# markokr/libacm

Hardware: AMD Instinct MI355X
Metric: decoded PCM Msamples/sec over a batch of ACM streams (hot path on HBM-resident staged input) (higher is better)
Workload: dtype int32

## Files before the change

libacm_amd/_build.py:

```python
import os
import shutil
import subprocess

ROOT = os.path.dirname(os.path.dirname(os.path.abspath(__file__)))
PKG = os.path.join(ROOT, "libacm_amd")
CSRC = os.path.join(PKG, "csrc")
LIB = os.path.join(PKG, "lib")
BIN = os.path.join(PKG, "bin")
INC = os.path.join(ROOT, "include")

HIPCC = os.environ.get("HIPCC") or shutil.which("hipcc") or "/opt/rocm/bin/hipcc"
GFX = "gfx950"


def _stale(target, sources):
    if not os.path.exists(target):
        return True
    t = os.path.getmtime(target)
    return any(os.path.getmtime(s) > t for s in sources if os.path.exists(s))


def _run(cmd):
    r = subprocess.run(cmd, stdout=subprocess.PIPE, stderr=subprocess.STDOUT, text=True)
    if r.returncode != 0:
        raise RuntimeError("build step failed: %s\n%s" % (" ".join(cmd), r.stdout))
    return r.stdout


def _headers():
    return [os.path.join(INC, f) for f in os.listdir(INC)] + \
           [os.path.join(CSRC, f) for f in os.listdir(CSRC) if f.endswith((".h", ".hpp", ".inc"))]


def build_synth(force=False):
    os.makedirs(LIB, exist_ok=True)
    out = os.path.join(LIB, "libacmsynth.so")
    src = [os.path.join(CSRC, "acm_synth.c")]
    if force or _stale(out, src + _headers()):
        _run(["gcc", "-O2", "-g", "-Wall", "-Wextra", "-fPIC", "-shared", "-I", INC, "-o", out] + src)
    return out


HIP_SOURCES = ["acm_kernels.hip", "acm_kernels_f32.hip", "acm_parse.hip", "acm_hip_api.cpp", "acm_fill.cpp", "acm_pack.cpp", "acm_stream.cpp", "acm_batch.cpp",
               "acm_host_synth.cpp", "acm_plan_cut.cpp", "acm_index.cpp", "acm_batch_windows.cpp", "acm_batch_layout.cpp"]
HOST_ONLY = {"acm_host_synth.cpp", "acm_plan_cut.cpp", "acm_index.cpp", "acm_batch_layout.cpp"}
INCLUDES = {"acm_kernels_f32.hip": ["acm_kernels.hip"]}


def build_hip(force=False):
    os.makedirs(LIB, exist_ok=True)
    out = os.path.join(LIB, "libacm_hip.so")
    src = [os.path.join(CSRC, f) for f in HIP_SOURCES if os.path.exists(os.path.join(CSRC, f))]
    if force or _stale(out, src + _headers()):
        objs = []
        for s in src:
            o = os.path.join(LIB, os.path.basename(s) + ".o")
            deps = [os.path.join(CSRC, f) for f in INCLUDES.get(os.path.basename(s), [])]
            if force or _stale(o, [s] + deps + _headers()):
                cmd = [HIPCC, "-O3", "-g1", "-std=c++17", "-fPIC", "-Wall", "-Wextra",
                       "--offload-arch=" + GFX, "-I", INC, "-I", CSRC, "-c", s, "-o", o]
                if os.environ.get("ACM_ABLATION"):
                    cmd.insert(1, "-DACM_ABLATION=1")
                if os.environ.get("ACM_TUNING"):
                    cmd.insert(1, "-DACM_TUNING=1")
                extra = os.environ.get("ACM_HIPCC_EXTRA", "").split()
                cmd[1:1] = extra
                if os.path.basename(s) in HOST_ONLY:
                    cmd = [c for c in cmd if not c.startswith("--offload-arch")]
                elif s.endswith(".cpp"):
                    cmd.insert(1, "-x")
                    cmd.insert(2, "hip")
                _run(cmd)
            objs.append(o)
        _run([HIPCC, "-shared", "-fPIC", "--offload-arch=" + GFX, "-o", out] + objs + ["-lpthread"])
    return out


def build_tuning(force=False):
# ... 55 lines not shown
```

libacm_amd/csrc/acm_device.h:

```cpp
#ifndef ACM_DEVICE_H
#define ACM_DEVICE_H

#include <stdint.h>

#include "acm_hip.h"

struct AcmDevStream {
	uint64_t idx_off;
	uint64_t hdr_off;
	uint64_t pcm_off;
	uint64_t n_emit;
	uint64_t scratch_off;
	uint32_t level;
	uint32_t rows;
	uint32_t nrows;
	uint32_t row_begin;
	uint32_t halo_row;
	uint32_t pad;
};

struct AcmTile {
	uint32_t stream;
	int32_t row0;
	uint32_t flags;
// ... 85 lines not shown
int acmhip_aux_stream(acmhip_device *dev, int k, void **out);
int acmhip_report_hip(int hip_error, const char *what);
void acmhip_set_error_text(const char *text);

#define ACMK_FMT_F32 0x100u
int acmk_tuning_build(void);
int acmk_warmup(void *stream);
int acmk_fused_variants(void);
int acmk_fused_tile_rows(uint32_t level, int variant);
int acmk_fused_has_carry(uint32_t level, int variant);
int acmk_fused_grid(uint32_t level, int variant, int cus);
int acmk_launch_fused(uint32_t level, int variant, int cus, int carry, const AcmDevStream *d_streams, const AcmTile *d_tiles,
		      uint32_t ntiles, const int16_t *d_idx, const acmhip_blkhdr *d_hdr, int16_t *d_pcm, unsigned fmt, void *stream);
int acmk_tile2_rows(uint32_t level);
int acmk_tile2_grid(uint32_t level, int cus);
#define ACM_K2_SINK_BYTES 65536
#define ACM_K2_SINK_F32_BYTES (2 * ACM_K2_SINK_BYTES)
int acmk_launch_tile2(uint32_t level, int cus, const AcmTile2 *d_tiles, uint32_t ntiles, const int16_t *d_idx, const acmhip_blkhdr *d_hdr, int16_t *d_pcm,
		      int16_t *d_sink, unsigned fmt, void *stream);
int acmk_tile2p_rows(uint32_t level);
int acmk_tile2p_group_rows(uint32_t level);
int acmk_tile2p_slots(uint32_t level);
int acmk_tile2p_waves(uint32_t level);
int acmk_tile2p_pad_shift(uint32_t level);
int acmk_launch_tile2p(uint32_t level, int cus, const AcmTile2 *d_tiles, uint32_t ntiles, const acmhip_packed_chunk *d_chunks, const uint8_t *d_blob,
		       const acmhip_blkhdr *d_hdr, int16_t *d_pcm, int16_t *d_sink, unsigned fmt, void *stream);
int acmk_tile2m_rows(uint32_t level);
int acmk_tile2m_lead_in(uint32_t level);
int acmk_tile2m_run_waves(uint32_t level, int cus);
int acmk_tile2m_grid(uint32_t level, int cus);
int acmk_tile2m_stages(uint32_t level);
int acmk_launch_tile2m(uint32_t level, int cus, const AcmTile2 *d_tiles, uint32_t ntiles, const uint8_t *d_mform, const acmhip_mform_pair *d_pairs,
		       const acmhip_blkhdr *d_hdr, int16_t *d_pcm, int16_t *d_sink, unsigned fmt, void *stream);
int acmk_launch_unpack(const AcmDevStream *d_streams, const uint32_t *d_list, uint32_t nlist, uint64_t max_elems,
		       const int16_t *d_idx, const acmhip_blkhdr *d_hdr, int32_t *d_x, uint32_t shift, void *stream);
int acmk_launch_prefix(const AcmDevStream *d_streams, const uint32_t *d_list, uint32_t nlist, uint64_t max_elems,
		       uint32_t level, const int16_t *d_idx, const acmhip_blkhdr *d_hdr, int32_t *d_y, void *stream);
int acmk_plane_tile_rows(void);
int acmk_plane_grid(int cus);
int acmk_launch_fused_plane(int cus, int carry, const AcmDevStream *d_streams, const AcmTile *d_tiles, uint32_t ntiles,
			    const int32_t *d_plane, int16_t *d_pcm, unsigned fmt, void *stream);
int acmk_launch_patch(const AcmDevPatch *d_patches, uint64_t n, int32_t *d_x, void *stream);
int acmk_launch_stage(const AcmDevStream *d_streams, const uint32_t *d_list, uint32_t nlist, uint64_t max_elems,
		      uint32_t level, uint32_t k, const int32_t *d_in, int32_t *d_out, uint32_t shift, void *stream);
int acmk_parse_supported(uint32_t level, uint32_t rows, uint64_t file_len, uint64_t blocks);
int acmk_launch_parse(const AcmParseJob *d_jobs, uint32_t njobs, const uint8_t *d_files, uint32_t *d_colpos, int16_t *d_idx,
		      acmhip_blkhdr *d_hdr, AcmParseResult *d_res, uint32_t *d_flags, uint64_t max_columns, void *stream);
#define ACM_PARSE_RANGE_MAX_STREAMS 32768
int acmk_launch_parse_range(const AcmParseJob *d_jobs, uint32_t njobs, const uint8_t *d_files, uint32_t *d_colpos, int16_t *d_idx,
			    acmhip_blkhdr *d_hdr, AcmParseResult *d_res, uint32_t *d_flags, uint64_t max_columns, uint32_t r, uint32_t R,
			    uint32_t stripes_up, void *stream);
int acmk_launch_parse_range_mf(const AcmParseJob *d_jobs, uint32_t njobs, const uint8_t *d_files, uint32_t *d_colpos, int16_t *d_idx,
			       acmhip_blkhdr *d_hdr, AcmParseResult *d_res, uint32_t *d_flags, uint64_t max_columns, uint32_t r, uint32_t R,
			       uint32_t stripes_up, uint8_t *d_mf, uint32_t *d_pairs, uint32_t *d_blkoff, void *stream);
int acmk_launch_parse_blocks(const AcmParseJob *d_jobs, uint32_t njobs, const AcmBlockJob *d_bjobs, uint32_t nblock, const uint8_t *d_files,
			     uint32_t *d_colpos, int16_t *d_idx, acmhip_blkhdr *d_hdr, AcmParseResult *d_res, uint32_t *d_flags,
			     uint64_t max_columns, void *stream);
uint32_t acmk_stripe_bound(uint32_t file_len, uint32_t s, uint32_t S);
uint32_t acmk_range_bound(uint32_t blocks, uint32_t r, uint32_t R, uint32_t unit);
int acmk_launch_scatter_stripe(const AcmParseJob *d_jobs, uint32_t njobs, const uint64_t *d_stripe_at, const uint8_t *d_stage,
			       uint8_t *d_files, uint32_t s, uint32_t S, void *stream);
int acmk_launch_small(uint32_t level, const AcmDevStream *d_streams, const uint32_t *d_list, uint32_t nlist, uint64_t max_emit,
		      const int16_t *d_idx, const acmhip_blkhdr *d_hdr, int16_t *d_pcm, unsigned fmt, void *stream);
int acmk_launch_emit(const AcmDevStream *d_streams, const uint32_t *d_list, uint32_t nlist, uint64_t max_emit,
		     const int32_t *d_x, int16_t *d_pcm, unsigned fmt, void *stream);
int acmk_launch_fused_f32(uint32_t level, int variant, int cus, int carry, const AcmDevStream *d_streams, const AcmTile *d_tiles,
// ... 17 lines not shown
```

libacm_amd/csrc/acm_kernels.hip:

```cpp
#include <hip/hip_runtime.h>

#include <utility>

#include "acm_device.h"

#ifndef ACM_L14_GROUPS
#define ACM_L14_GROUPS 3, 3, 3, 3, 2
#endif
#ifndef ACM_L13_GROUPS
#define ACM_L13_GROUPS 2, 3, 3, 3, 2
#endif

#ifndef ACM_OUT_F32
#define ACM_OUT_F32 0
#endif
#if ACM_OUT_F32
#define ACM_K_EMIT acm_sw_emit_f32
#define ACM_K_SMALL acm_small_level_f32
#define ACM_K_FUSED acm_fused_tile_f32
#define ACM_K_TILE2 acm_f32_tile2
#define ACM_K_CHUNK acm_f32_chunk
#define ACMK_OUT(name) name##_f32
#else
#define ACM_K_EMIT acm_sw_emit
#define ACM_K_SMALL acm_small_level
#define ACM_K_FUSED acm_fused_tile
#define ACM_K_TILE2 acm_tile2
#define ACM_K_CHUNK acm_chunk
#define ACMK_OUT(name) name
#endif

namespace {

__device__ __forceinline__ uint32_t pcm16(int32_t v, int level, unsigned fmt)
{
	uint32_t w = (uint32_t)(v >> level);
	if (fmt & 2u)
// ... 1978 lines not shown
#ifndef ACM_K3_DPP_HISTORY
#define ACM_K3_DPP_HISTORY 1
#endif
	static constexpr bool HISTORY_BY_DPP = ACM_K3_DPP_HISTORY && RR >= 2 && NSW == 2 && RR * SIGMA == 16 && SIGMA >= 4;
	static constexpr bool KEEPS_ROWS = HISTORY_IN_REGISTERS || HISTORY_BY_DPP;
	template <int CTRL, int BANKS>
	static __device__ __forceinline__ v4u_t dpp4(const v4u_t old, const v4u_t src)
	{
		v4u_t r;
#pragma unroll
		for (int v = 0; v < 4; v++)
			r[v] = (uint32_t)__builtin_amdgcn_update_dpp((int)old[v], (int)src[v], CTRL, 0xF, BANKS, false);
		return r;
	}
	static constexpr int DPP_W0_BANKS = (1 << (SIGMA / 4)) - 1;
	static __device__ __forceinline__ void hand_history_on(Raw &raw)
	{
#pragma unroll
		for (int k = 0; k < 2; k++) {
			raw.lo[0][k] = dpp4<0x100 + (16 - SIGMA), DPP_W0_BANKS>(raw.lo[0][k], raw.lo[0][k + NSW]);
			raw.hi[0][k] = dpp4<0x100 + (16 - SIGMA), DPP_W0_BANKS>(raw.hi[0][k], raw.hi[0][k + NSW]);
		}
	}
	static __device__ __forceinline__ void take_history_from_partner(Raw &raw)
	{
#pragma unroll
		for (int k = 0; k < 2; k++) {
			raw.lo[0][k] = dpp4<0x110 + SIGMA, 0xF & ~DPP_W0_BANKS>(raw.lo[0][k], raw.lo[0][k + NSW]);
			raw.hi[0][k] = dpp4<0x110 + SIGMA, 0xF & ~DPP_W0_BANKS>(raw.hi[0][k], raw.hi[0][k + NSW]);
		}
	}
	static constexpr int JM = (TR & 1) ? 1 : TR / 2;
	static_assert(JM + 1 <= NE, "entries in reach are entries fetched");
	static __device__ __forceinline__ uint32_t half_bytes(const uint32_t cls) { return (0x4234u >> (4u * cls)) & 15u; }
	template <int J0>
	static __device__ __forceinline__ uint32_t mode_of(const uint32_t flags, const Desc &d, const uint32_t sval)
	{
		const uint32_t cls = d.e[0] & 3u;
		const uint32_t pair_units = (uint32_t)(COLS / 64) * half_bytes(cls);
		bool ok = (flags & ACM_TILE_ONEBLOCK) != 0 && cls != 0u;
		if constexpr (OutScale<L>::SHIFT != 0)
			ok = ok && sval < 65536u;
#pragma unroll
		for (int j = 1; j <= JM; j++)
			ok = ok && (d.e[j] & 3u) == cls;
#pragma unroll
		for (int j = J0; j < JM; j++)
			ok = ok && (d.e[j + 1] >> 2) - (d.e[j] >> 2) == pair_units;
		return ok ? (cls == ACMHIP_BP_NIB12 ? 3u : cls - (ACMHIP_BP_BYTE - 1u)) : 0u;
	}

#ifndef ACM_K3_LD_MOD
#define ACM_K3_LD_MOD " nt"
#endif
	template <bool KEEP>
	static __device__ __forceinline__ void issue(Raw &raw, const uint8_t *arena, const Desc &d, const int lane, const uint32_t odd, const uint32_t mode)
	{
		static_assert(!KEEP || KEEPS_ROWS, "the rows in front belong to another lane");
		constexpr int K0 = KEEP ? 2 : 0, J0 = KEEP ? 1 : 0;
		const uint32_t i = (uint32_t)lane & 15u, ks = (uint32_t)lane >> 4;
		const uint32_t c = class_of(i), rr = RR == 1 ? 0u : i / SIGMA;
		const uint32_t smode = __builtin_amdgcn_readfirstlane(mode);
		uint32_t va[NX][NG], vh[NX][NG];
		const uint8_t *sb[NX][NG];
		if (mode) {
			const uint32_t hb = smode == 1u ? 2u : smode == 2u ? 4u : 3u;
			const uint64_t base = reinterpret_cast<uint64_t>(arena) + ((uint64_t)(d.e[J0] >> 2) << 6);
			const uint32_t vl = (rr * (uint32_t)(NSW * COLS / 2) + c * (uint32_t)(QN / 2)) * hb + 16u * ks;
			const uint32_t vlh = vl - (smode == 3u ? 8u * ks : 0u);
#pragma unroll
			for (int k = K0; k < NX; k++)
#pragma unroll
				for (int g = 0; g < NG; g++) {
					va[k][g] = vl;
					vh[k][g] = vlh;
					sb[k][g] = sgpr_u64(base + (uint64_t)((((TR & 1 ? odd : 0u) + (uint32_t)(k - K0)) * (uint32_t)(COLS / 2) + group_at(g) * (uint32_t)(QN / 2)) * hb));
				}
		} else {
			const uint32_t e0 = d.e[0];
			const uint8_t *base = sgpr_u64(reinterpret_cast<uint64_t>(arena) + ((uint64_t)(e0 >> 2) << 6));
#pragma unroll
			for (int k = K0; k < NX; k++) {
				const uint32_t u = (TR & 1 ? odd : 0u) + rr * NSW + k;
				const uint32_t e = entry_of(d, u);
				const uint32_t hb = half_bytes(e & 3u);
				const uint32_t row_at = (((e >> 2) - (e0 >> 2)) << 6) + ((u & 1u) ? (uint32_t)(COLS / 2) * hb : 0u) + 16u * ks;
#pragma unroll
				for (int g = 0; g < NG; g++) {
					va[k][g] = row_at + (group_at(g) + c) * (uint32_t)(QN / 2) * hb;
					vh[k][g] = va[k][g] - ((e & 3u) == ACMHIP_BP_NIB12 ? 8u * ks : 0u);
					sb[k][g] = base;
				}
			}
		}
#pragma unroll
// ... 40 lines not shown
		for (int g = 0; g < NG; g++)
#pragma unroll
			for (int k = 0; k < 2; k++) {
				raw.lo[g][k] = raw.lo[g][k + NSW];
				raw.hi[g][k] = raw.hi[g][k + NSW];
			}
	}
	static __device__ __forceinline__ void zero_history(Raw &raw)
	{
		const v4u_t z = { 0, 0, 0, 0 };
#pragma unroll
		for (int g = 0; g < NG; g++)
#pragma unroll
			for (int k = 0; k < 2; k++)
				raw.lo[g][k] = raw.hi[g][k] = z;
	}

	static __device__ __forceinline__ v4i_t mfma(const v4u_t data, const v4i_t coef, const v4i_t acc)
	{
		return __builtin_amdgcn_mfma_i32_16x16x64_i8((v4i_t)data, coef, acc, 0, 0, 0);
	}

	static __device__ __forceinline__ int32_t opaque_s(int32_t v)
	{
		asm("" : "+s"(v));
		return v;
	}
	static __device__ __forceinline__ int32_t opaque_v(int32_t v)
	{
		asm("" : "+v"(v));
		return v;
	}

	template <bool WORDS, bool FAST, bool NIB = false>
	static __device__ __forceinline__ void run_t(const Raw &raw, uint32_t *const tile, const Tables &t, const int lane, const uint32_t hvs,
						     const uint32_t in_front, const uint32_t sval, const bool wordu = false, const Desc *dd = nullptr,
						     const uint32_t odd = 0u, const bool nform = false)
	{
		static_assert(!NIB || (WORDS && FAST), "rows in N form are a fast-path matter; the general path takes them to bytes first");
		const v4i_t zero = { 0, 0, 0, 0 };
		const uint32_t h = (uint32_t)lane >> 4, qd = (uint32_t)lane & 15u;
		uint32_t c0[NH], rrd[NH];
		uint32_t o_lane[NH];
#pragma unroll
		for (int hf = 0; hf < NH; hf++) {
			const uint32_t i = 4u * h + (uint32_t)(hf * NVH);
			c0[hf] = RR == 1 ? class_of(i) : i % SIGMA;
			rrd[hf] = RR == 1 ? 0u : i / SIGMA;
			const uint32_t m_lane = rrd[hf] * (uint32_t)(NSW * COLS) + c0[hf] + (uint32_t)SIGMA * qd;
			o_lane[hf] = m_lane + (m_lane >> PS);
		}
		uint32_t bias_at[NSW][NH];
		int32_t val[NSW][NH], dv2[NSW][NH], dv1[NSW][NH];
		bool step2[NSW], step1[NSW];
		bool small[NSW];
#pragma unroll
		for (int s = 0; s < NSW; s++)
			small[s] = OutScale<L>::SHIFT == 0;
		if constexpr (FAST) {
#pragma unroll
			for (int s = 0; s < NSW; s++) {
				step2[s] = step1[s] = false;
				small[s] = true;
#pragma unroll
				for (int hf = 0; hf < NH; hf++)
					val[s][hf] = dv2[s][hf] = dv1[s][hf] = 0;
			}
		} else if constexpr (RR <= 2) {
			int32_t rowval[TR + 2];
#pragma unroll
			for (int k = 0; k < TR + 2; k++)
				rowval[k] = (int32_t)__builtin_amdgcn_readlane(hvs, k);
// ... 18 lines not shown
				}
			}
		} else {
			const uint32_t first = (uint32_t)__builtin_amdgcn_readfirstlane(hvs);
			const bool one_val = __builtin_amdgcn_ballot_w64(lane < TR + 2 && hvs != first) == 0;
#pragma unroll
			for (int s = 0; s < NSW; s++)
				step2[s] = step1[s] = false;
#pragma unroll
			for (int hf = 0; hf < NH; hf++) {
				int32_t g[NSW + 2];
#pragma unroll
				for (int k = 0; k < NSW + 2; k++)
					g[k] = one_val ? (int32_t)first : __builtin_amdgcn_ds_bpermute((int)(4u * (rrd[hf] * NSW + (uint32_t)k)), (int32_t)hvs);
#pragma unroll
				for (int s = 0; s < NSW; s++) {
					val[s][hf] = g[s + 2];
					dv2[s][hf] = g[s + 1] - g[s + 2];
					dv1[s][hf] = g[s] - g[s + 1];
					if (!one_val) {
						step2[s] = step2[s] || __builtin_amdgcn_ballot_w64(dv2[s][hf] != 0) != 0;
						step1[s] = step1[s] || __builtin_amdgcn_ballot_w64(dv1[s][hf] != 0) != 0;
					}
				}
			}
		}
#pragma unroll
		for (int s = 0; s < NSW; s++)
#pragma unroll
			for (int hf = 0; hf < NH; hf++) {
				const uint32_t row = in_front + rrd[hf] * NSW + s;
				bias_at[s][hf] = ((row < 2 ? row : 2u) * 2u + (c0[hf] == 0 ? 0u : 1u)) * (uint32_t)QN + qd;
			}
		const v4i_t *cf = &t.coef[0][0][lane];
		const auto &hi = raw.hi;
#ifndef ACM_K3_MT_UNROLL
#define ACM_K3_MT_UNROLL 1
#endif
#define ACM_PRAGMA_(x) _Pragma(#x)
#define ACM_UNROLL(n) ACM_PRAGMA_(unroll n)
		ACM_UNROLL(ACM_K3_MT_UNROLL)
		for (int mt = 0; mt < NM; mt++) {
			const v4i_t cf0 = cf[0], cf1 = cf[NM * 64], cf2 = cf[2 * NM * 64];
#pragma unroll
			for (int e = 0; e < NSET; e++) {
				const int g = e / NSW, s = e % NSW;
				int32_t b[NH];
#pragma unroll
				for (int hf = 0; hf < NH; hf++)
					b[hf] = g == 0 ? (&t.bias[0][0][0])[bias_at[s][hf] + 16u * (uint32_t)mt] : 0;
				const v4i_t l1 = mfma(raw.lo[g][s], cf2, zero);
				const v4i_t l2 = mfma(raw.lo[g][s + 1], cf1, l1);
				const v4i_t la = mfma(raw.lo[g][s + 2], cf0, l2);
				v4i_t y;
				if constexpr (FAST) {
					const int32_t sv = opaque_s((int32_t)__builtin_amdgcn_readfirstlane(sval));
#pragma unroll
					for (int v = 0; v < 4; v++)
						y[v] = __mul24(la[v], sv) + (v % NVH == 0 ? b[v / NVH] : 0);
					if constexpr (WORDS) {
						const v4i_t h1 = mfma(hi[g][s], cf2, zero);
						const v4i_t h2 = mfma(hi[g][s + 1], cf1, h1);
						const v4i_t ha = mfma(hi[g][s + 2], cf0, h2);
						if constexpr (NIB) {
							const int32_t sv4 = opaque_s((int32_t)__builtin_amdgcn_readfirstlane(sval << 4));
#pragma unroll
							for (int v = 0; v < 4; v++)
								y[v] = __mul24(ha[v], sv4) + y[v];
						} else {
							const uint32_t sv8 = (uint32_t)opaque_s((int32_t)__builtin_amdgcn_readfirstlane(sval << 8));
#pragma unroll
							for (int v = 0; v < 4; v++)
								y[v] = (int32_t)(__umul24((uint32_t)ha[v], sv8) + (uint32_t)y[v]);
						}
					}
				} else {
#pragma unroll
				for (int v = 0; v < 4; v++)
					y[v] = __mul24(la[v], val[s][v / NVH]) + (v % NVH == 0 ? b[v / NVH] : 0);
				if (step2[s]) {
#pragma unroll
					for (int v = 0; v < 4; v++)
						y[v] += __mul24(l2[v], dv2[s][v / NVH]);
				}
				if (step1[s]) {
#pragma unroll
					for (int v = 0; v < 4; v++)
						y[v] += __mul24(l1[v], dv1[s][v / NVH]);
				}
				if constexpr (WORDS && NH == 1) {
					if (wordu) {
						const int32_t *rs = &t.rsum[0][0] + 16 * mt + (int)qd;
						bool urow[3];
#pragma unroll
						for (int j = 0; j < 3; j++)
							urow[j] = (entry_of(*dd, (TR & 1 ? odd : 0u) + rrd[0] * NSW + (uint32_t)(s + j)) & 3u) == ACMHIP_BP_WORDU;
						const int32_t v0 = val[s][0], v1 = v0 + dv2[s][0], v2 = v1 + dv1[s][0];
// ... 38 lines not shown
					}
					if (step1[s]) {
#pragma unroll
						for (int v = 0; v < 4; v++)
							yh[v] += __mul24(h1[v], w1[v / NVH]);
					}
					const uint32_t hs = nform ? 4u : 8u;
#pragma unroll
					for (int v = 0; v < 4; v++)
						y[v] = (int32_t)(((uint32_t)opaque_v(yh[v]) << hs) + (uint32_t)y[v]);
					}
				joined:;
				}
				}
				static_assert(COLS % (1 << PS) == 0 && (SIGMA * 16) % (1 << PS) == 0 &&
					      (NG == 1 || (group_at(NG - 1) % (1 << PS) + CB + 7 < (1 << PS) && SIGMA % (1 << PS) == 0)), "address split");
#pragma unroll
				for (int hf = 0; hf < NH; hf++) {
					uint32_t *const o = tile + (o_lane[hf] + (uint32_t)((s * COLS + ((s * COLS) >> PS)) + (group_at(g) + (group_at(g) >> PS))));
#pragma unroll
					for (int v = 0; v < NVH; v++)
						o[v] = (uint32_t)y[hf * NVH + v];
				}
			}
			cf += 64;
#pragma unroll
			for (int hf = 0; hf < NH; hf++)
				o_lane[hf] += SIGMA * 16 + ((SIGMA * 16) >> PS);
		}
	}

	static __device__ __forceinline__ void run(Raw &raw, uint32_t *const tile, const Tables &t, const int lane_, const uint32_t hvs,
						   const Desc &d, const uint32_t in_front, const uint32_t odd, const uint32_t mode, const uint32_t sval,
						   const bool first)
	{
#ifdef ACM_K3_OPAQUE_LANE
		const int lane = opaque_v(lane_);
#else
		const int lane = lane_;
#endif
		const bool all_new = !KEEPS_ROWS || first;
		if (mode == 3u) {
#pragma unroll
			for (int k = 0; k < NX; k++)
				if (k >= 2 || all_new) {
#pragma unroll
					for (int g = 0; g < NG; g++)
						raw.hi[g][k] = expand_nib(raw.hi[g][k]);
				}
			if constexpr (HISTORY_BY_DPP)
				take_history_from_partner(raw);
			run_t<true, true, true>(raw, tile, t, lane, 0u, in_front, sval);
			return;
		}
		if (mode) {
			if constexpr (HISTORY_BY_DPP)
				take_history_from_partner(raw);
			if (mode == 2u)
				run_t<true, true>(raw, tile, t, lane, 0u, in_front, sval);
			else
				run_t<false, true>(raw, tile, t, lane, 0u, in_front, sval);
			return;
		}
		uint32_t any_word = 0, any_nib = 0, any_wordu = 0;
#pragma unroll
		for (int j = 0; j < NE; j++) {
			any_word |= (d.e[j] & 3u) == ACMHIP_BP_WORD ? 1u : 0u;
			any_nib |= (d.e[j] & 3u) == ACMHIP_BP_NIB12 ? 1u : 0u;
			any_wordu |= (d.e[j] & 3u) == ACMHIP_BP_WORDU ? 1u : 0u;
		}
		any_word |= any_wordu;
		const uint32_t rr = RR == 1 ? 0u : ((uint32_t)lane & 15u) / SIGMA;
		if (any_nib) {
#pragma unroll
			for (int k = 0; k < NX; k++)
				if (k >= 2 || all_new) {
					if ((entry_of(d, (TR & 1 ? odd : 0u) + rr * NSW + k) & 3u) == ACMHIP_BP_NIB12) {
#pragma unroll
						for (int g = 0; g < NG; g++)
							raw.hi[g][k] = expand_nib(raw.hi[g][k]);
					}
				}
		}
		if constexpr (HISTORY_BY_DPP)
			take_history_from_partner(raw);
		const bool nform = any_nib && !any_word;
		if (any_word | any_nib) {
#pragma unroll
			for (int k = 0; k < NX; k++) {
				const uint32_t cls = entry_of(d, (TR & 1 ? odd : 0u) + rr * NSW + k) & 3u;
				const uint32_t mask = cls == ACMHIP_BP_BYTE ? 0u : 0xFFFFFFFFu;
#pragma unroll
				for (int g = 0; g < NG; g++)
					raw.hi[g][k] &= mask;
				if (any_nib && !nform && cls == ACMHIP_BP_NIB12) {
#pragma unroll
					for (int g = 0; g < NG; g++)
						raw.hi[g][k] = sra4(raw.hi[g][k]);
				}
// ... 48 lines not shown
		return;
	bool discard = false;
	{
		const uint32_t f0 = tiles[__builtin_amdgcn_readfirstlane(t)].flags;
		if (f0 & ACM_TILE_DISCARD) {
			discard = true;
		} else if (!(f0 & ACM_TILE_FRESH)) {
			discard = true;
			t--;
		}
	}

	auto rows_in_front = [](const AcmTile2 &r) -> uint32_t { return (r.flags & ACM_TILE_FRESH) ? 0u : (r.flags & ACM_TILE_ROW1) ? 1u : 2u; };
	auto fetch_val = [&](const AcmTile2 &r, const int lane, uint32_t v, const uint32_t mode) -> uint32_t {
		const uint32_t *p = &hdr[0].val;
		if (!mode) {
			const uint32_t lr_fetch = (uint32_t)(lane < TR + 2 ? lane : TR + 1);
			const uint32_t missing = 2u - rows_in_front(r);
			const uint32_t q = r.rowpos + (lr_fetch < missing ? 0u : lr_fetch - missing);
			const uint32_t b = r.magic ? __umulhi(q, r.magic) : q;
			p = &hdr[r.hdr_blk + b].val;
		}
		asm volatile("s_cmp_lg_u32 %2, 0\n\ts_cbranch_scc1 .Lacm_zv_%=\n\t"
			     "global_load_dword %0, %1, off\n"
			     ".Lacm_zv_%=:"
			     : "+v"(v) : "v"(p), "s"(__builtin_amdgcn_readfirstlane(mode)) : "memory", "scc");
		return v;
	};
	typedef const uint32_t __attribute__((address_space(4))) *const_u32_ptr;
	auto val_of = [&](const AcmTile2 &r) -> uint32_t {
		const uint64_t a = reinterpret_cast<uint64_t>(&hdr[__builtin_amdgcn_readfirstlane(r.hdr_blk)].val);
		return *(const_u32_ptr)a << OutScale<L>::SHIFT;
	};

	constexpr int NVEC = TR * COLS / 8, PER_OWNER = NJ_LAST / 8, NSTORE = NVEC / 64;
	static_assert(NVEC % 64 == 0, "whole rounds");
	const uint8_t *const arena = reinterpret_cast<const uint8_t *>(idx);
	auto record_at = [&](const uint32_t k) -> AcmTile2 { return tiles[__builtin_amdgcn_readfirstlane(k < t_end ? k : t_end - 1)]; };
	constexpr int MODE_J0 = FP::KEEPS_ROWS ? 1 : 0;
#ifdef ACM_K3_NO_FAST
	auto mode_of = [&](const AcmTile2 &, const typename FP::Desc &, const uint32_t) -> uint32_t { return 0u; };
#else
	auto mode_of = [&](const AcmTile2 &r, const typename FP::Desc &d, const uint32_t sval) -> uint32_t {
		return FP::template mode_of<MODE_J0>(r.flags, d, sval);
	};
#endif
	AcmTile2 cur = record_at(t);
	typename FP::Desc dcur = FP::fetch_desc(pairs, cur);
	typename FP::Raw raw;
	{
		const v4u_t z = { 0, 0, 0, 0 };
#pragma unroll
		for (int g = 0; g < FP::NG; g++)
#pragma unroll
			for (int k = 0; k < FP::NX; k++)
				raw.hi[g][k] = z;
	}
	uint32_t mode_cur = 0u, sv_cur = val_of(cur);
	uint32_t hv = fetch_val(cur, lane0, 0u, 0u);
	FP::template issue<false>(raw, arena, dcur, lane0, (cur.flags & ACM_TILE_ODD) ? 1u : 0u, 0u);
	k2_wait<0>();
	bool fresh = true, first_of_run = true;
	AcmTile2 nxt = record_at(t + 1), nx2 = record_at(t + 2);
	typename FP::Desc dnxt = FP::fetch_desc(pairs, nxt);
	uint32_t sv_nxt = val_of(nxt);
	uint32_t mode_nxt = mode_of(nxt, dnxt, sv_nxt);
#ifdef ACM_STAMPS
	unsigned long long acc_[8] = { 0, 0, 0, 0, 0, 0, 0, 0 };
	unsigned long long last_ = stamp_now();
#endif
	for (;;) {
		const uint32_t tn = t + 1;
		const bool more = tn < t_end;
		int lane = lane0;
#ifdef ACM_K3_OPAQUE_LANE
		asm volatile("" : "+v"(lane));
#endif
		if (fresh)
			for (int k = lane; k < NCARRY_WORDS; k += 64)
				carry_mem[k] = 0u;
		const uint32_t hvs = hv << OutScale<L>::SHIFT;
		ACM_STAMP(0);
		phase_prio<true, PRIO_FIRST_PASS>();
		FP::run(raw, tile, tables, lane, hvs, dcur, rows_in_front(cur), (cur.flags & ACM_TILE_ODD) ? 1u : 0u, mode_cur, sv_cur, first_of_run);
		first_of_run = false;
		phase_prio<true, PRIO_IDLE>();
		ACM_STAMP(1);

		hv = fetch_val(nxt, lane, hv, mode_nxt);
		if constexpr (FP::HISTORY_IN_REGISTERS) {
			FP::shift_history(raw);
			if (nxt.flags & ACM_TILE_FRESH)
				FP::zero_history(raw);
			FP::template issue<true>(raw, arena, dnxt, lane, (nxt.flags & ACM_TILE_ODD) ? 1u : 0u, mode_nxt);
		} else if constexpr (FP::HISTORY_BY_DPP) {
			FP::hand_history_on(raw);
			if (nxt.flags & ACM_TILE_FRESH)
				FP::zero_history(raw);
			FP::template issue<true>(raw, arena, dnxt, lane, (nxt.flags & ACM_TILE_ODD) ? 1u : 0u, mode_nxt);
		} else {
			FP::template issue<false>(raw, arena, dnxt, lane, (nxt.flags & ACM_TILE_ODD) ? 1u : 0u, mode_nxt);
		}
		const AcmTile2 nx3 = record_at(t + 3);
		const typename FP::Desc dnx2 = FP::fetch_desc(pairs, nx2);
		const uint32_t sv_nx2 = val_of(nx2);
		ACM_STAMP(2);
		phase_prio<true, PRIO_LDS_PASSES>();
		run_lds_passes<C, PASS_ABL, true, FP::G, Gs...>(tile, lane, F32 ? (unsigned)ACMHIP_FMT_S16LE : fmt, carry_mem);
		tile_barrier<MODE_WAVE>();
		ACM_STAMP(3);
		if constexpr (F32) {
			float *out = discard ? reinterpret_cast<float *>(sink) : reinterpret_cast<float *>(pcm) + cur.pcm_off;
			lean_store_f32<C, 64, NSTORE, ABL>(tile, lane, out);
		} else {
			typedef uint32_t v4u __attribute__((ext_vector_type(4)));
			v4u *out = discard ? reinterpret_cast<v4u *>(sink) : reinterpret_cast<v4u *>(reinterpret_cast<uint16_t *>(pcm) + cur.pcm_off);
#pragma unroll
			for (int k = 0; k < NSTORE; k++) {
				const int vec = lane + k * 64;
				const uint32_t *q = tile + lds_at<C::PS>((vec / PER_OWNER) * NJ_LAST) + (vec % PER_OWNER) * park_piece<NJ_LAST>();
				const v4u o = { q[0], q[1], q[2], q[3] };
#ifdef ACM_K3_ST_MOD
				asm volatile("global_store_dwordx4 %0, %1, %2" ACM_K3_ST_MOD :: "v"((uint32_t)(vec * 16)), "v"(o), "s"(sgpr_u64(reinterpret_cast<uint64_t>(out))) : "memory");
#else
				__builtin_nontemporal_store(o, &out[vec]);
#endif
			}
		}
		ACM_STAMP(5);
		phase_prio<true, PRIO_IDLE>();
		k2_wait<F32 ? 2 * NSTORE : NSTORE>();
		ACM_STAMP(6);
		tile_barrier<MODE_WAVE>();
		if (!more)
			break;
		fresh = (nxt.flags & (ACM_TILE_FRESH | ACM_TILE_DISCARD)) != 0;
		discard = (nxt.flags & ACM_TILE_DISCARD) != 0;
		cur = nxt;
		dcur = dnxt;
		sv_cur = sv_nxt;
		mode_cur = mode_nxt;
		t = tn;
		nxt = nx2;
		dnxt = dnx2;
		sv_nxt = sv_nx2;
		mode_nxt = mode_of(nxt, dnxt, sv_nxt);
		nx2 = nx3;
	}
#ifdef ACM_STAMPS
	if (lane0 == 0 && vw < 2048)
		for (int k = 0; k < 8; k++)
			g_acm_stamps[vw][k] = acc_[k];
#endif
}

struct Tile2Entry {
	typedef void (*Fn)(const AcmTile2 *, uint32_t, const int16_t *, const uint32_t *, const acmhip_blkhdr *, int16_t *, int16_t *, unsigned);
	Fn fn;
	int threads, tile_rows, wg_per_cu;
};
template <class C, int... Gs>
constexpr Tile2Entry entry_k2()
{
	return Tile2Entry{ ACM_K_TILE2<C, 4, 0, false, Gs...>, C::NT, C::TR, 1024 / C::NT };
}
template <class C, int WPC, int... Gs>
constexpr Tile2Entry entry_k2w()
{
	return Tile2Entry{ ACM_K_TILE2<C, WPC * C::NT / 256, 0, false, Gs...>, C::NT, C::TR, WPC };
}
#ifdef ACM_ABLATION
template <int ABL>
constexpr Tile2Entry abl_k2() { return Tile2Entry{ ACM_K_TILE2<TileCfg<9, 256, 8192>, 4, ABL, false, 3, 3, 3>, 256, 16, 4 }; }
const struct { int mask; Tile2Entry e; } g_tile2_abl[] = {
	{ 1, abl_k2<1>() }, { 2, abl_k2<2>() }, { 4, abl_k2<4>() }, { 6, abl_k2<6>() }, { 8, abl_k2<8>() }, { 16, abl_k2<16>() },
	{ 17, abl_k2<17>() }, { 23, abl_k2<23>() }, { 32, abl_k2<32>() }, { 25, abl_k2<25>() }, { 31, abl_k2<31>() }, { 12, abl_k2<12>() },
};
#endif
const Tile2Entry g_tile2[ACM_K2_MAX_LEVEL - ACM_K2_MIN_LEVEL + 1] = {
// ... 750 lines not shown
```

Baseline: 1.432 million.

## Add fast path for chunks that straddle a block start at levels 8 and 9

Adds a shared host/device classifier that recognises tiles which begin exactly at a block boundary with compatible packing classes on both sides. Those tiles now take a fast MFMA decode path instead of the general path. The scale difference between the two blocks is applied as a correction to the first rows, and the high plane of the front rows is zeroed or expanded as needed. A second header value is now loaded per tile, and the new arithmetic in the inner loop may add register pressure and code size. A host entry point exposes the same classifier, apparently for checking.

```diff
diff --git a/libacm_amd/_build.py b/libacm_amd/_build.py
--- a/libacm_amd/_build.py
+++ b/libacm_amd/_build.py
@@ -42,8 +42,8 @@
 
 
 HIP_SOURCES = ["acm_kernels.hip", "acm_kernels_f32.hip", "acm_parse.hip", "acm_hip_api.cpp", "acm_fill.cpp", "acm_pack.cpp", "acm_stream.cpp", "acm_batch.cpp",
-               "acm_host_synth.cpp", "acm_plan_cut.cpp", "acm_index.cpp", "acm_batch_windows.cpp", "acm_batch_layout.cpp"]
-HOST_ONLY = {"acm_host_synth.cpp", "acm_plan_cut.cpp", "acm_index.cpp", "acm_batch_layout.cpp"}
+               "acm_host_synth.cpp", "acm_plan_cut.cpp", "acm_index.cpp", "acm_batch_windows.cpp", "acm_batch_layout.cpp", "acm_chunk_path.cpp"]
+HOST_ONLY = {"acm_host_synth.cpp", "acm_plan_cut.cpp", "acm_index.cpp", "acm_batch_layout.cpp", "acm_chunk_path.cpp"}
 INCLUDES = {"acm_kernels_f32.hip": ["acm_kernels.hip"]}
 
 
diff --git a/libacm_amd/csrc/acm_chunk_path.cpp b/libacm_amd/csrc/acm_chunk_path.cpp
--- /dev/null
+++ b/libacm_amd/csrc/acm_chunk_path.cpp
@@ -0,0 +1,30 @@
+#include "acm_chunk_path.h"
+
+namespace {
+
+template <int L>
+uint32_t path_at(const AcmTile2 *rec, const uint32_t *pairs, const acmhip_blkhdr *hdr)
+{
+	using Geo = AcmChunkGeo<L>;
+	uint32_t e[Geo::NE];
+	for (int j = 0; j < Geo::NE; j++)
+		e[j] = pairs[rec->idx_off + (uint64_t)j];
+	const uint32_t oneblock = (rec->flags & ACM_TILE_ONEBLOCK) ? 1u : 0u;
+	const uint32_t sval_p = hdr[rec->hdr_blk].val << Geo::SHIFT;
+	const uint32_t sval_c = hdr[rec->hdr_blk + (oneblock ? 0u : 1u)].val << Geo::SHIFT;
+	return acm_chunk_path_of<L, 1>(rec->flags, rec->rowpos, rec->magic, e, sval_p, sval_c);
+}
+
+}
+
+extern "C" uint32_t acmk_chunk_path(uint32_t level, const AcmTile2 *rec, const uint32_t *pairs, const acmhip_blkhdr *hdr)
+{
+	switch (level) {
+	case 8: return path_at<8>(rec, pairs, hdr);
+	case 9: return path_at<9>(rec, pairs, hdr);
+	case 10: return path_at<10>(rec, pairs, hdr);
+	case 11: return path_at<11>(rec, pairs, hdr);
+	case 12: return path_at<12>(rec, pairs, hdr);
+	default: return 0u;
+	}
+}
diff --git a/libacm_amd/csrc/acm_chunk_path.h b/libacm_amd/csrc/acm_chunk_path.h
--- /dev/null
+++ b/libacm_amd/csrc/acm_chunk_path.h
@@ -0,0 +1,95 @@
+#ifndef ACM_CHUNK_PATH_H
+#define ACM_CHUNK_PATH_H
+
+#include <stdint.h>
+
+#include "acm_device.h"
+
+#ifdef __HIP__
+#define ACM_PATH_FN __attribute__((host)) __attribute__((device)) inline __attribute__((always_inline))
+#else
+#define ACM_PATH_FN static inline
+#endif
+
+#ifdef __clang__
+#define ACM_PATH_UNROLL _Pragma("unroll")
+#else
+#define ACM_PATH_UNROLL
+#endif
+
+#define ACM_PATH_OWN(p)   ((p) & 3u)
+#define ACM_PATH_FRONT(p) ((p) >> 2)
+
+template <int L>
+struct AcmChunkGeo {
+	static constexpr int COLS = 1 << L;
+	static constexpr int NELEM = COLS > 2048 ? COLS : 2048;
+	static constexpr int TR = NELEM / COLS;
+	static constexpr int JM = (TR & 1) ? 1 : TR / 2;
+	static constexpr int NE = JM + 1;
+	static constexpr int SHIFT = (L <= 8) ? 8 - L : (L >= 10 ? 16 - L : 0);
+	static constexpr bool BLOCK_START = (L == 8 || L == 9);
+};
+
+ACM_PATH_FN uint32_t acm_path_half_bytes(const uint32_t cls) { return (0x4234u >> (4u * cls)) & 15u; }
+ACM_PATH_FN uint32_t acm_path_mode_of_class(const uint32_t cls)
+{
+	return cls == ACMHIP_BP_WORDU ? 0u : cls == ACMHIP_BP_NIB12 ? 3u : cls - (ACMHIP_BP_BYTE - 1u);
+}
+ACM_PATH_FN uint32_t acm_path_mulhi(const uint32_t a, const uint32_t b) { return (uint32_t)(((uint64_t)a * b) >> 32); }
+
+template <int L, int J0>
+ACM_PATH_FN bool acm_path_one_width(const uint32_t (&e)[AcmChunkGeo<L>::NE], const uint32_t cls, bool ok)
+{
+	constexpr int JM = AcmChunkGeo<L>::JM;
+	const uint32_t pair_units = (uint32_t)(AcmChunkGeo<L>::COLS / 64) * acm_path_half_bytes(cls);
+	ACM_PATH_UNROLL
+	for (int j = 1; j <= JM; j++)
+		ok = ok && (e[j] & 3u) == cls;
+	ACM_PATH_UNROLL
+	for (int j = J0; j < JM; j++)
+		ok = ok && (e[j + 1] >> 2) - (e[j] >> 2) == pair_units;
+	return ok;
+}
+
+template <int L, int J0>
+ACM_PATH_FN uint32_t acm_chunk_mode(const uint32_t flags, const uint32_t (&e)[AcmChunkGeo<L>::NE], const uint32_t sval)
+{
+	const bool own_only = AcmChunkGeo<L>::BLOCK_START && J0 == 1 && (flags & ACM_TILE_FRESH) != 0;
+	const uint32_t cls = (own_only ? e[1] : e[0]) & 3u;
+	bool ok = (flags & ACM_TILE_ONEBLOCK) != 0 && cls != ACMHIP_BP_WORDU;
+	if (AcmChunkGeo<L>::SHIFT != 0)
+		ok = ok && sval < 65536u;
+	ok = acm_path_one_width<L, J0>(e, cls, ok);
+	return ok ? (cls == ACMHIP_BP_NIB12 ? 3u : cls - (ACMHIP_BP_BYTE - 1u)) : 0u;
+}
+
+template <int L>
+ACM_PATH_FN bool acm_chunk_starts_block(const uint32_t flags, const uint32_t rowpos, const uint32_t magic)
+{
+	if (flags & (ACM_TILE_ONEBLOCK | ACM_TILE_FRESH | ACM_TILE_ROW1 | ACM_TILE_ODD))
+		return false;
+	if (magic == 0u || rowpos >= 65536u)
+		return false;
+	return acm_path_mulhi(rowpos + 1u, magic) == 0u && acm_path_mulhi(rowpos + 2u, magic) == 1u &&
+	       acm_path_mulhi(rowpos + 1u + (uint32_t)AcmChunkGeo<L>::TR, magic) == 1u;
+}
+
+template <int L, int J0>
+ACM_PATH_FN uint32_t acm_chunk_path_of(const uint32_t flags, const uint32_t rowpos, const uint32_t magic, const uint32_t (&e)[AcmChunkGeo<L>::NE],
+				       const uint32_t sval_p, const uint32_t sval_c)
+{
+	if (flags & ACM_TILE_ONEBLOCK)
+		return acm_chunk_mode<L, J0>(flags, e, sval_p);
+	if (!AcmChunkGeo<L>::BLOCK_START || !acm_chunk_starts_block<L>(flags, rowpos, magic))
+		return 0u;
+	const uint32_t front = e[0] & 3u, own = e[1] & 3u;
+	bool ok = front != ACMHIP_BP_WORDU && own != ACMHIP_BP_WORDU;
+	ok = ok && !((front == ACMHIP_BP_NIB12 && own == ACMHIP_BP_WORD) || (front == ACMHIP_BP_WORD && own == ACMHIP_BP_NIB12));
+	ok = ok && (sval_p | sval_c) < 65536u;
+	ok = acm_path_one_width<L, 1>(e, own, ok);
+	return ok ? acm_path_mode_of_class(own) | front << 2 : 0u;
+}
+
+
+#endif
diff --git a/libacm_amd/csrc/acm_device.h b/libacm_amd/csrc/acm_device.h
--- a/libacm_amd/csrc/acm_device.h
+++ b/libacm_amd/csrc/acm_device.h
@@ -141,6 +141,7 @@
 int acmk_tile2m_stages(uint32_t level);
 int acmk_launch_tile2m(uint32_t level, int cus, const AcmTile2 *d_tiles, uint32_t ntiles, const uint8_t *d_mform, const acmhip_mform_pair *d_pairs,
 		       const acmhip_blkhdr *d_hdr, int16_t *d_pcm, int16_t *d_sink, unsigned fmt, void *stream);
+uint32_t acmk_chunk_path(uint32_t level, const AcmTile2 *rec, const uint32_t *pairs, const acmhip_blkhdr *hdr);
 int acmk_launch_unpack(const AcmDevStream *d_streams, const uint32_t *d_list, uint32_t nlist, uint64_t max_elems,
 		       const int16_t *d_idx, const acmhip_blkhdr *d_hdr, int32_t *d_x, uint32_t shift, void *stream);
 int acmk_launch_prefix(const AcmDevStream *d_streams, const uint32_t *d_list, uint32_t nlist, uint64_t max_elems,
diff --git a/libacm_amd/csrc/acm_kernels.hip b/libacm_amd/csrc/acm_kernels.hip
--- a/libacm_amd/csrc/acm_kernels.hip
+++ b/libacm_amd/csrc/acm_kernels.hip
@@ -3,6 +3,7 @@
 #include <utility>
 
 #include "acm_device.h"
+#include "acm_chunk_path.h"
 
 #ifndef ACM_L14_GROUPS
 #define ACM_L14_GROUPS 3, 3, 3, 3, 2
@@ -2047,22 +2048,18 @@
 	}
 	static constexpr int JM = (TR & 1) ? 1 : TR / 2;
 	static_assert(JM + 1 <= NE, "entries in reach are entries fetched");
-	static __device__ __forceinline__ uint32_t half_bytes(const uint32_t cls) { return (0x4234u >> (4u * cls)) & 15u; }
+	using Geo = AcmChunkGeo<L_>;
+	static_assert(Geo::COLS == COLS && Geo::TR == TR && Geo::JM == JM && Geo::NE == NE && Geo::SHIFT == OutScale<L_>::SHIFT, "one geometry");
+	static constexpr bool BLOCK_START = Geo::BLOCK_START && HISTORY_BY_DPP && NSW == 2 && NH == 1 && NG == 1;
+	static_assert(BLOCK_START || !Geo::BLOCK_START || !ACM_K3_DPP_HISTORY, "the host's classifier and the kernel agree on the levels");
+	static __device__ __forceinline__ uint32_t half_bytes(const uint32_t cls) { return acm_path_half_bytes(cls); }
 	template <int J0>
-	static __device__ __forceinline__ uint32_t mode_of(const uint32_t flags, const Desc &d, const uint32_t sval)
-	{
-		const uint32_t cls = d.e[0] & 3u;
-		const uint32_t pair_units = (uint32_t)(COLS / 64) * half_bytes(cls);
-		bool ok = (flags & ACM_TILE_ONEBLOCK) != 0 && cls != 0u;
-		if constexpr (OutScale<L>::SHIFT != 0)
-			ok = ok && sval < 65536u;
-#pragma unroll
-		for (int j = 1; j <= JM; j++)
-			ok = ok && (d.e[j] & 3u) == cls;
-#pragma unroll
-		for (int j = J0; j < JM; j++)
-			ok = ok && (d.e[j + 1] >> 2) - (d.e[j] >> 2) == pair_units;
-		return ok ? (cls == ACMHIP_BP_NIB12 ? 3u : cls - (ACMHIP_BP_BYTE - 1u)) : 0u;
+	static __device__ __forceinline__ uint32_t mode_of(const AcmTile2 &r, const Desc &d, const uint32_t sval, const uint32_t sval2)
+	{
+		if constexpr (BLOCK_START)
+			return acm_chunk_path_of<L_, J0>(r.flags, r.rowpos, r.magic, d.e, sval, sval2);
+		else
+			return acm_chunk_mode<L_, J0>(r.flags, d.e, sval);
 	}
 
 #ifndef ACM_K3_LD_MOD
@@ -2075,7 +2072,7 @@
 		constexpr int K0 = KEEP ? 2 : 0, J0 = KEEP ? 1 : 0;
 		const uint32_t i = (uint32_t)lane & 15u, ks = (uint32_t)lane >> 4;
 		const uint32_t c = class_of(i), rr = RR == 1 ? 0u : i / SIGMA;
-		const uint32_t smode = __builtin_amdgcn_readfirstlane(mode);
+		const uint32_t smode = BLOCK_START ? ACM_PATH_OWN(__builtin_amdgcn_readfirstlane(mode)) : __builtin_amdgcn_readfirstlane(mode);
 		uint32_t va[NX][NG], vh[NX][NG];
 		const uint8_t *sb[NX][NG];
 		if (mode) {
@@ -2182,12 +2179,13 @@
 		return v;
 	}
 
-	template <bool WORDS, bool FAST, bool NIB = false>
+	template <bool WORDS, bool FAST, bool NIB = false, bool BS = false>
 	static __device__ __forceinline__ void run_t(const Raw &raw, uint32_t *const tile, const Tables &t, const int lane, const uint32_t hvs,
 						     const uint32_t in_front, const uint32_t sval, const bool wordu = false, const Desc *dd = nullptr,
-						     const uint32_t odd = 0u, const bool nform = false)
+						     const uint32_t odd = 0u, const bool nform = false, const uint32_t sdv = 0u)
 	{
 		static_assert(!NIB || (WORDS && FAST), "rows in N form are a fast-path matter; the general path takes them to bytes first");
+		static_assert(!BS || (FAST && !NIB && BLOCK_START), "a chunk that starts a block: one fast flavour, the shift of its high plane a scalar");
 		const v4i_t zero = { 0, 0, 0, 0 };
 		const uint32_t h = (uint32_t)lane >> 4, qd = (uint32_t)lane & 15u;
 		uint32_t c0[NH], rrd[NH];
@@ -2272,6 +2270,11 @@
 				const uint32_t row = in_front + rrd[hf] * NSW + s;
 				bias_at[s][hf] = ((row < 2 ? row : 2u) * 2u + (c0[hf] == 0 ? 0u : 1u)) * (uint32_t)QN + qd;
 			}
+		int32_t dvl = 0, dvh = 0;
+		if constexpr (BS) {
+			dvl = rrd[0] == 0u ? (int32_t)__builtin_amdgcn_readfirstlane(sdv) : 0;
+			dvh = opaque_v(dvl);
+		}
 		const v4i_t *cf = &t.coef[0][0][lane];
 		const auto &hi = raw.hi;
 #ifndef ACM_K3_MT_UNROLL
@@ -2298,11 +2301,35 @@
 #pragma unroll
 					for (int v = 0; v < 4; v++)
 						y[v] = __mul24(la[v], sv) + (v % NVH == 0 ? b[v / NVH] : 0);
+					if constexpr (BS) {
+						if (s < 2) {
+							const v4i_t lx = s == 0 ? l2 : l1;
+#pragma unroll
+							for (int v = 0; v < 4; v++)
+								y[v] = __mul24(lx[v], dvl) + y[v];
+						}
+					}
 					if constexpr (WORDS) {
 						const v4i_t h1 = mfma(hi[g][s], cf2, zero);
 						const v4i_t h2 = mfma(hi[g][s + 1], cf1, h1);
 						const v4i_t ha = mfma(hi[g][s + 2], cf0, h2);
-						if constexpr (NIB) {
+						if constexpr (BS) {
+							const int32_t svh = opaque_s((int32_t)__builtin_amdgcn_readfirstlane(sval));
+							const v4i_t hx = s == 0 ? h2 : h1;
+							v4i_t yh;
+#pragma unroll
+							for (int v = 0; v < 4; v++)
+								yh[v] = __mul24(ha[v], svh);
+							if (s < 2) {
+#pragma unroll
+								for (int v = 0; v < 4; v++)
+									yh[v] = __mul24(hx[v], dvh) + yh[v];
+							}
+							const uint32_t hs = nform ? 4u : 8u;
+#pragma unroll
+							for (int v = 0; v < 4; v++)
+								y[v] = (int32_t)(((uint32_t)opaque_v(yh[v]) << hs) + (uint32_t)y[v]);
+						} else if constexpr (NIB) {
 							const int32_t sv4 = opaque_s((int32_t)__builtin_amdgcn_readfirstlane(sval << 4));
 #pragma unroll
 							for (int v = 0; v < 4; v++)
@@ -2407,7 +2434,7 @@
 
 	static __device__ __forceinline__ void run(Raw &raw, uint32_t *const tile, const Tables &t, const int lane_, const uint32_t hvs,
 						   const Desc &d, const uint32_t in_front, const uint32_t odd, const uint32_t mode, const uint32_t sval,
-						   const bool first)
+						   const bool first, const uint32_t sval2 = 0u)
 	{
 #ifdef ACM_K3_OPAQUE_LANE
 		const int lane = opaque_v(lane_);
@@ -2415,6 +2442,34 @@
 		const int lane = lane_;
 #endif
 		const bool all_new = !KEEPS_ROWS || first;
+		if constexpr (BLOCK_START) {
+			if (ACM_PATH_FRONT(mode)) {
+				const uint32_t own = ACM_PATH_OWN(mode), front = ACM_PATH_FRONT(mode);
+				const bool planes = own != 1u || front != ACMHIP_BP_BYTE;
+				const v4u_t z = { 0, 0, 0, 0 };
+				if (own == 3u) {
+#pragma unroll
+					for (int k = 2; k < NX; k++)
+						raw.hi[0][k] = expand_nib(raw.hi[0][k]);
+				} else if (own == 1u && planes) {
+#pragma unroll
+					for (int k = 2; k < NX; k++)
+						raw.hi[0][k] = z;
+				}
+				if (front == ACMHIP_BP_BYTE && planes) {
+#pragma unroll
+					for (int k = 0; k < 2; k++)
+						raw.hi[0][k] = z;
+				}
+				take_history_from_partner(raw);
+				const bool nform = own == 3u || front == ACMHIP_BP_NIB12;
+				if (planes)
+					run_t<true, true, false, true>(raw, tile, t, lane, 0u, in_front, sval2, false, nullptr, 0u, nform, sval - sval2);
+				else
+					run_t<false, true, false, true>(raw, tile, t, lane, 0u, in_front, sval2, false, nullptr, 0u, false, sval - sval2);
+				return;
+			}
+		}
 		if (mode == 3u) {
 #pragma unroll
 			for (int k = 0; k < NX; k++)
@@ -2439,7 +2494,7 @@
 		}
 		uint32_t any_word = 0, any_nib = 0, any_wordu = 0;
 #pragma unroll
-		for (int j = 0; j < NE; j++) {
+		for (int j = 0; j <= JM; j++) {
 			any_word |= (d.e[j] & 3u) == ACMHIP_BP_WORD ? 1u : 0u;
 			any_nib |= (d.e[j] & 3u) == ACMHIP_BP_NIB12 ? 1u : 0u;
 			any_wordu |= (d.e[j] & 3u) == ACMHIP_BP_WORDU ? 1u : 0u;
@@ -2554,6 +2609,11 @@
 		const uint64_t a = reinterpret_cast<uint64_t>(&hdr[__builtin_amdgcn_readfirstlane(r.hdr_blk)].val);
 		return *(const_u32_ptr)a << OutScale<L>::SHIFT;
 	};
+	auto val2_of = [&](const AcmTile2 &r) -> uint32_t {
+		const uint32_t b = __builtin_amdgcn_readfirstlane(r.hdr_blk) + ((__builtin_amdgcn_readfirstlane(r.flags) & ACM_TILE_ONEBLOCK) ? 0u : 1u);
+		const uint64_t a = reinterpret_cast<uint64_t>(&hdr[b].val);
+		return *(const_u32_ptr)a << OutScale<L>::SHIFT;
+	};
 
 	constexpr int NVEC = TR * COLS / 8, PER_OWNER = NJ_LAST / 8, NSTORE = NVEC / 64;
 	static_assert(NVEC % 64 == 0, "whole rounds");
@@ -2561,10 +2621,10 @@
 	auto record_at = [&](const uint32_t k) -> AcmTile2 { return tiles[__builtin_amdgcn_readfirstlane(k < t_end ? k : t_end - 1)]; };
 	constexpr int MODE_J0 = FP::KEEPS_ROWS ? 1 : 0;
 #ifdef ACM_K3_NO_FAST
-	auto mode_of = [&](const AcmTile2 &, const typename FP::Desc &, const uint32_t) -> uint32_t { return 0u; };
+	auto mode_of = [&](const AcmTile2 &, const typename FP::Desc &, const uint32_t, const uint32_t) -> uint32_t { return 0u; };
 #else
-	auto mode_of = [&](const AcmTile2 &r, const typename FP::Desc &d, const uint32_t sval) -> uint32_t {
-		return FP::template mode_of<MODE_J0>(r.flags, d, sval);
+	auto mode_of = [&](const AcmTile2 &r, const typename FP::Desc &d, const uint32_t sval, const uint32_t sval2) -> uint32_t {
+		return FP::template mode_of<MODE_J0>(r, d, sval, sval2);
 	};
 #endif
 	AcmTile2 cur = record_at(t);
@@ -2585,8 +2645,8 @@
 	bool fresh = true, first_of_run = true;
 	AcmTile2 nxt = record_at(t + 1), nx2 = record_at(t + 2);
 	typename FP::Desc dnxt = FP::fetch_desc(pairs, nxt);
-	uint32_t sv_nxt = val_of(nxt);
-	uint32_t mode_nxt = mode_of(nxt, dnxt, sv_nxt);
+	uint32_t sv_nxt = val_of(nxt), sc_cur = 0u, sc_nxt = FP::BLOCK_START ? val2_of(nxt) : 0u;
+	uint32_t mode_nxt = mode_of(nxt, dnxt, sv_nxt, sc_nxt);
 #ifdef ACM_STAMPS
 	unsigned long long acc_[8] = { 0, 0, 0, 0, 0, 0, 0, 0 };
 	unsigned long long last_ = stamp_now();
@@ -2604,7 +2664,7 @@
 		const uint32_t hvs = hv << OutScale<L>::SHIFT;
 		ACM_STAMP(0);
 		phase_prio<true, PRIO_FIRST_PASS>();
-		FP::run(raw, tile, tables, lane, hvs, dcur, rows_in_front(cur), (cur.flags & ACM_TILE_ODD) ? 1u : 0u, mode_cur, sv_cur, first_of_run);
+		FP::run(raw, tile, tables, lane, hvs, dcur, rows_in_front(cur), (cur.flags & ACM_TILE_ODD) ? 1u : 0u, mode_cur, sv_cur, first_of_run, sc_cur);
 		first_of_run = false;
 		phase_prio<true, PRIO_IDLE>();
 		ACM_STAMP(1);
@@ -2625,7 +2685,7 @@
 		}
 		const AcmTile2 nx3 = record_at(t + 3);
 		const typename FP::Desc dnx2 = FP::fetch_desc(pairs, nx2);
-		const uint32_t sv_nx2 = val_of(nx2);
+		const uint32_t sv_nx2 = val_of(nx2), sc_nx2 = FP::BLOCK_START ? val2_of(nx2) : 0u;
 		ACM_STAMP(2);
 		phase_prio<true, PRIO_LDS_PASSES>();
 		run_lds_passes<C, PASS_ABL, true, FP::G, Gs...>(tile, lane, F32 ? (unsigned)ACMHIP_FMT_S16LE : fmt, carry_mem);
@@ -2661,12 +2721,14 @@
 		cur = nxt;
 		dcur = dnxt;
 		sv_cur = sv_nxt;
+		sc_cur = sc_nxt;
 		mode_cur = mode_nxt;
 		t = tn;
 		nxt = nx2;
 		dnxt = dnx2;
 		sv_nxt = sv_nx2;
-		mode_nxt = mode_of(nxt, dnxt, sv_nxt);
+		sc_nxt = sc_nx2;
+		mode_nxt = mode_of(nxt, dnxt, sv_nxt, sc_nxt);
 		nx2 = nx3;
 	}
 #ifdef ACM_STAMPS
```

After: 1.417 million. -1.1%, worse.
